# Mr-wang27/llm-inference

Measured on AMD Instinct MI355X. Metric: decode tokens/sec Llama-2-7B fp16 @1 GPU; % HBM roofline; 1->8 TP curve, higher is better.
Workload: dtype fp16; 1 GPU; Llama-2-7B fp16 single-stream greedy decode to 2048 tokens (BASELINE.json configs[1]); TP over n_gpus when > 1; batch=1, prompt=8, ctx=1..2048, kv_cache=f16, weights=fp16, fp32 activations/accumulate, parallelism=single

## Files before the change

### llm-inference_amd/csrc/attn.hip

```cpp
#include <cstdlib>

#include "attn_impl.h"
#include "xchg_impl.h"

namespace llmi {
namespace {

using namespace attn_detail;

template <typename KT, bool HOST_SIZED>
__global__ __launch_bounds__(kThreads) void attn_decode_kernel(AttnArgs a, int ns) {
    extern __shared__ __attribute__((aligned(16))) float smem[];
    WgStamp ts(a.stamps);
    attn_body<KT, PlainIO, HOST_SIZED>(a, blockIdx.x, blockIdx.y, ns, smem, &ts);
}

__global__ __launch_bounds__(kThreads) void attn_merge_kernel(AttnArgs a, int ns) {
    __shared__ float m_s[kMaxSplits];
    __shared__ float l_s[kMaxSplits];
    __shared__ float red_s[16];
    __shared__ float o_red[2][D];
    const int pos = a.pos_dev ? *a.pos_dev : a.pos_host;
    const int h = blockIdx.x, tid = threadIdx.x;
    const int d = tid % D, half = tid / D;
    Ws ws = ws_carve(a.workspace, a.heads, ns);
    const float* mlh = ws.ml + (size_t)h * ns * 2;
    const float* oh = ws.o + (size_t)h * ns * D + d;
    float ov[kMergeChunk];
#pragma unroll
// ... 16 lines not shown
    const float L = block_sum(lw, red_s);
    float O = 0.f;
#pragma unroll
    for (int i = 0; i < kMergeChunk; ++i) {
        const int sp = half + 2 * i;
        const float w = sp < nact ? expf(m_s[sp] - M) : 0.f;
        O = fmaf(sp < nact ? ov[i] : 0.f, w, O);
    }
    for (int sp = half + 2 * kMergeChunk; sp < nact; sp += 2) O = fmaf(oh[(size_t)sp * D], expf(m_s[sp] - M), O);
    o_red[half][d] = O;
    __syncthreads();
    if (tid < D) a.out[(size_t)h * D + tid] = (o_red[0][tid] + o_red[1][tid]) / L;
}

template <typename WT, int NPL>
__global__ __launch_bounds__(kThreads) void attn_oproj_kernel(OprojArgs a, int ns) {
    extern __shared__ __attribute__((aligned(16))) float smem[];
    WgStamp ts(a.stamps);
    oproj_body<WT, NPL, PlainIO>(a, blockIdx.x, blockIdx.y, ns, smem);
    xchg_detail::xchg_tail(a.xt, a.xt_cnt, reinterpret_cast<int*>(smem));
}

template <typename WT, int NPL>
__global__ __launch_bounds__(kThreads) void attn_oproj2_kernel(OprojArgs a, int ns) {
    extern __shared__ __attribute__((aligned(16))) float smem[];
    WgStamp ts(a.stamps);
    oproj_body2<WT, NPL, PlainIO>(a, blockIdx.x, blockIdx.y, ns, smem);
    xchg_detail::xchg_tail(a.xt, a.xt_cnt, reinterpret_cast<int*>(smem));
}

#ifndef LLMI_OPROJ_HG
#define LLMI_OPROJ_HG 2
#endif

int oproj_npl(const OprojArgs& a) {
    const long target = (long)a.heads * a.n_rows / (1024 * 16);
#ifdef LLMI_OPROJ_NPL
    if (target >= 8) return LLMI_OPROJ_NPL;
#endif
    return target >= 8 ? 8 : target >= 4 ? 4 : target >= 2 ? 2 : 1;
}

template <typename WT>
int oproj_launch_w(const OprojArgs& a, hipStream_t s) {
    const int ns = (a.max_seq + CH - 1) / CH;
    const int npl = oproj_npl(a);
    if (LLMI_OPROJ_HG == 2 && sizeof(WT) == 2 && a.heads % 2 == 0 && !a.head_major && npl == 8) {
        const dim3 grid2(a.heads / 2, (a.n_rows + 8 * npl - 1) / (8 * npl));
        hipLaunchKernelGGL((attn_oproj2_kernel<WT, 8>), grid2, dim3(kThreads), oproj2_lds<8>(), s, a, ns);
        LLMI_HIP(hipGetLastError());
        return LLMI_OK;
    }
    const dim3 grid(a.heads, (a.n_rows + 16 * npl - 1) / (16 * npl));
    switch (npl) {
#if LLMI_OPROJ_NPL == 16
        case 16: hipLaunchKernelGGL((attn_oproj_kernel<WT, 16>), grid, dim3(kThreads), oproj_lds<16>(), s, a, ns); break;
#endif
        case 8: hipLaunchKernelGGL((attn_oproj_kernel<WT, 8>), grid, dim3(kThreads), oproj_lds<8>(), s, a, ns); break;
        case 4: hipLaunchKernelGGL((attn_oproj_kernel<WT, 4>), grid, dim3(kThreads), oproj_lds<4>(), s, a, ns); break;
        case 2: hipLaunchKernelGGL((attn_oproj_kernel<WT, 2>), grid, dim3(kThreads), oproj_lds<2>(), s, a, ns); break;
        default: hipLaunchKernelGGL((attn_oproj_kernel<WT, 1>), grid, dim3(kThreads), oproj_lds<1>(), s, a, ns); break;
    }
    LLMI_HIP(hipGetLastError());
    return LLMI_OK;
}

}

size_t attn_workspace_bytes(int heads, int head_dim, int max_seq) {
    (void)head_dim;
    return ws_bytes(heads, max_seq);
}

int attn_decode_launch(const AttnArgs& a, hipStream_t s) {
    LLMI_REQUIRE(a.head_dim == D, "attn: head_dim must be 128");
    LLMI_REQUIRE(a.heads > 0 && a.kv_heads > 0 && a.heads % a.kv_heads == 0, "attn: bad head counts");
    LLMI_REQUIRE(a.max_seq > 0 && (a.max_seq + CH - 1) / CH <= kMaxSplits, "attn: max_seq out of range");
    LLMI_REQUIRE(a.pos_dev || (a.pos_host >= 0 && a.pos_host < a.max_seq), "attn: pos out of range");
    LLMI_REQUIRE(a.qkv && a.k_cache && a.v_cache && a.workspace, "attn: null pointer");
    LLMI_REQUIRE(!a.direct_out || a.out, "attn: null output");
    LLMI_REQUIRE(!a.xacc || a.resid || a.resid_fixed, "attn: xacc seeding needs resid");
    const int ns = (a.max_seq + CH - 1) / CH;
    LLMI_REQUIRE(a.nact >= 0 && a.nact <= ns, "attn: nact out of range");
    LLMI_REQUIRE(a.pos_dev || a.nact == 0 || a.nact == a.pos_host / CH + 1, "attn: nact != ceil((pos + 1) / 64)");
    LLMI_REQUIRE(a.nact == 0 || a.pos_dev, "attn: nact > 0 needs the device position");
    const bool hs = a.nact > 0;
    const dim3 grid(a.heads, hs ? a.nact : ns);
    if (a.cache_dtype == LLMI_F16) {
        if (hs)
            hipLaunchKernelGGL((attn_decode_kernel<__half, true>), grid, dim3(kThreads), kAttnLds, s, a, ns);
        else
            hipLaunchKernelGGL((attn_decode_kernel<__half, false>), grid, dim3(kThreads), kAttnLds, s, a, ns);
    } else if (a.cache_dtype == LLMI_F32) {
        if (hs)
            hipLaunchKernelGGL((attn_decode_kernel<float, true>), grid, dim3(kThreads), kAttnLds, s, a, ns);
        else
            hipLaunchKernelGGL((attn_decode_kernel<float, false>), grid, dim3(kThreads), kAttnLds, s, a, ns);
    } else {
        LLMI_REQUIRE(false, "attn: cache dtype must be f16 or f32");
    }
    LLMI_HIP(hipGetLastError());
    if (a.direct_out) {
        hipLaunchKernelGGL(attn_merge_kernel, dim3(a.heads), dim3(kThreads), 0, s, a, ns);
        LLMI_HIP(hipGetLastError());
    }
    return LLMI_OK;
}

int attn_oproj_launch(const OprojArgs& a, hipStream_t s) {
    LLMI_REQUIRE(a.head_dim == D, "attn_oproj: head_dim must be 128");
    LLMI_REQUIRE(a.w && a.workspace && a.xacc && a.heads > 0 && a.n_rows > 0, "attn_oproj: bad arguments");
    LLMI_REQUIRE(a.ldw >= a.heads * D, "attn_oproj: ldw < heads * head_dim");
// ... 15 lines not shown
```

### llm-inference_amd/csrc/attn_impl.h

```cpp
#pragma once
#include "io.h"
#include "kernels.h"

namespace llmi {
namespace attn_detail {


constexpr int kThreads = 256;
constexpr int D = 128;
#ifndef LLMI_ATTN_CH
#define LLMI_ATTN_CH 64
#endif
constexpr int CH = LLMI_ATTN_CH;
static_assert(CH % 64 == 0 && CH >= kAttnChunk, "chunk must be a multiple of 64");
constexpr int LPR = 16;

constexpr int NPG = CH / (kThreads / LPR);
constexpr int kMaxSplits = 1024;
constexpr int kMergeChunk = 16;
static_assert(kThreads == 2 * D, "merge maps two threads to each head dim");

__device__ __forceinline__ float block_max(float v, float* red) {
    const int lane = threadIdx.x & 63, w = threadIdx.x >> 6, nw = (blockDim.x + 63) >> 6;
    v = wave_max(v);
// ... 100 lines not shown
    } else {
        Raw<float> f;
        f.v[0] = r.v[0];
        f.v[1] = r.v[1];
        unpack8(f, v);
    }
}

constexpr size_t kAttnLds = (3 * D + CH + (kThreads / LPR) * D + 4) * sizeof(float);

__device__ __forceinline__ unsigned long long ld_granule(const unsigned long long* p) {
    return __hip_atomic_load(p, __ATOMIC_RELAXED, __HIP_MEMORY_SCOPE_AGENT);
}

template <typename KT, typename IO, bool HOST_SIZED = false, bool TAGGED = false>
__device__ __forceinline__ void attn_body(const AttnArgs& a, int h, int split, int ns, float* smem,
                                          const WgStamp* ts = nullptr) {
    static_assert(!TAGGED || HOST_SIZED, "the fused launch sizes the attention grid on the host");
    float* q_s = smem;
    float* kcur_s = q_s + D;
    float* vcur_s = kcur_s + D;
    float* p_s = vcur_s + D;
    float (*o_red)[D] = reinterpret_cast<float (*)[D]>(p_s + CH);
    float* ml_s = p_s + CH + (kThreads / LPR) * D;

    const int group = a.heads / a.kv_heads;
    const int kvh = h / group;
    const int tid = threadIdx.x;
    const int grp = tid / LPR, l16 = tid % LPR;
    const int start = split * CH;
    KT* kc = reinterpret_cast<KT*>(a.k_cache) + (size_t)kvh * a.max_seq * D;
// ... 243 lines not shown
        for (int i = h * per + tid; i < min((h + 1) * per, a.hidden); i += kThreads) {
            const bool pre = HOST_SIZED && a.resid_fixed && i == h * per + (int)tid;
            IO::st_ll(a.xacc + i, a.resid_scale == 0.f ? 0ll
                                  : pre            ? psd
                                  : a.resid_fixed  ? a.resid_fixed[i]
                                                   : to_fixed(a.resid[i]));
        }
    }
}


template <int NPL>
constexpr size_t oproj_lds() { return (2 * kMaxSplits + 4 + D + 2 * D + 16 * NPL) * sizeof(float); }

template <typename WT, int NPL>
__device__ __forceinline__ void oproj_load_w(const OprojArgs& a, int h, int chunk, W8<WT> (&wr)[NPL]) {
    const int grp = threadIdx.x / LPR, l16 = threadIdx.x % LPR;
    const int row0 = chunk * 16 * NPL;
    const WT* w = reinterpret_cast<const WT*>(a.w);
#pragma unroll
    for (int t = 0; t < NPL; ++t) {
        int row = row0 + grp + 16 * t;
        row = row < a.n_rows ? row : a.n_rows - 1;
        const size_t off = a.head_major ? ((size_t)h * a.n_rows + row) * D : (size_t)row * a.ldw + (size_t)h * D;
        if constexpr (sizeof(WT) == 1 && NPL >= 2) {
            if (t < NPL / 2) {
                int r2 = row0 + grp + 16 * (2 * t + (l16 >> 3));
                r2 = r2 < a.n_rows ? r2 : a.n_rows - 1;
                const size_t off2 =
                    a.head_major ? ((size_t)h * a.n_rows + r2) * D : (size_t)r2 * a.ldw + (size_t)h * D;
                wr[t].v[0] = ld_nt16(w + off2 + (l16 & 7) * 16);
            }
        } else {
            wr[t] = ld_w8<WT>(w + off + l16 * 8);
        }
    }
}

template <typename WT, int NPL, typename IO>
__device__ __forceinline__ void oproj_body(const OprojArgs& a, int h, int chunk, int ns, float* smem) {
    float* m_s = smem;
    float* l_s = m_s + kMaxSplits;
    float& linv_s = l_s[kMaxSplits];
    float* o_s = l_s + kMaxSplits + 4;
    float (*o_red)[D] = reinterpret_cast<float (*)[D]>(o_s + D);
    float* y_s = o_s + 3 * D;
    const int tid = threadIdx.x;
    const int grp = tid / LPR, l16 = tid % LPR;
    const int row0 = chunk * 16 * NPL;
    const WT* w = reinterpret_cast<const WT*>(a.w);

    Ws ws = ws_carve(const_cast<void*>(a.workspace), a.heads, ns);
    const int d = tid % D, half = tid / D;
    const float* mlh = ws.ml + (size_t)h * ns * 2;
    const float* oh = ws.o + (size_t)h * ns * D + d;
// ... 98 lines not shown
            atomicAdd(reinterpret_cast<unsigned long long*>(a.xacc + row), (unsigned long long)to_fixed(v));
        }
    }
}


template <int NPL>
constexpr size_t oproj2_lds() { return (4 * kMaxSplits + 4 + 2 * D + 2 * 8 * NPL) * sizeof(float); }

__device__ __forceinline__ float ld_wt(const float* p) {
    return __uint_as_float(__hip_atomic_load(reinterpret_cast<const unsigned*>(p), __ATOMIC_RELAXED,
                                             __HIP_MEMORY_SCOPE_AGENT));
}

template <typename WT, int NPL, typename IO, bool FUSED = false>
__device__ __forceinline__ void oproj_body2(const OprojArgs& a, int hp, int chunk, int ns, float* smem) {
    float* m_s = smem;
    float* l_s = m_s + 2 * kMaxSplits;
    float* linv_s = l_s + 2 * kMaxSplits;
    float* o_s = linv_s + 4;
    float* y_s = o_s + 2 * D;
    const int tid = threadIdx.x;
    const int grp = tid / LPR, l16 = tid % LPR;
    const int hs = grp >> 3, g8 = grp & 7;
    const int h = 2 * hp + hs;
    const int row0 = chunk * 8 * NPL;
    const WT* w = reinterpret_cast<const WT*>(a.w);

    Ws ws = ws_carve(const_cast<void*>(a.workspace), a.heads, ns);
    const int mh = tid >> 7, d = tid & (D - 1);
    const float* mlh = ws.ml + (size_t)(2 * hp + mh) * ns * 2;
// ... 162 lines not shown
```

### llm-inference_amd/csrc/common.h

```cpp
#pragma once
#include <hip/hip_runtime.h>
#include <hip/hip_fp16.h>
#include <cstdint>
#include <cstdio>
#include <cstring>
#include <string>
#include <stdexcept>

#include "../../include/llmi.h"

namespace llmi {

constexpr int kWave = 64;

void set_last_error(const std::string& msg);

struct Status {
    int code = LLMI_OK;
};

#define LLMI_HIP(expr)                                                                 \
    do {                                                                               \
        hipError_t _e = (expr);                                                        \
        if (_e != hipSuccess) {                                                        \
// ... 128 lines not shown

constexpr int kLo8Exp = 12;
__device__ __forceinline__ uint32_t lo8_pack4(float l0, float l1, float l2, float l3) {
    auto c = [](float v) { return fminf(fmaxf(v * (float)(1 << kLo8Exp), -448.f), 448.f); };
    int r = __builtin_amdgcn_cvt_pk_fp8_f32(c(l0), c(l1), 0, false);
    r = __builtin_amdgcn_cvt_pk_fp8_f32(c(l2), c(l3), r, true);
    return (uint32_t)r;
}

struct WgStamp {
    unsigned long long* p;
    unsigned long long t0;
    __device__ __forceinline__ explicit WgStamp(unsigned long long* base)
        : p(base ? base + 8 * ((size_t)blockIdx.x + (size_t)gridDim.x * blockIdx.y) : nullptr),
          t0(base ? __builtin_amdgcn_s_memrealtime() : 0ull) {}
    __device__ __forceinline__ void mark(int i) const {
        if (p && threadIdx.x == 0) p[i] = __builtin_amdgcn_s_memrealtime();
    }
    __device__ __forceinline__ ~WgStamp() {
        if (p && threadIdx.x == 0) {
            p[0] = t0;
            p[3] = __builtin_amdgcn_s_memrealtime();
            p[4] = __smid();
        }
    }
};

}
```

### llm-inference_amd/csrc/gemv_impl.h

```cpp
#pragma once
#include "io.h"
#include "kernels.h"

namespace llmi {
namespace gemv_detail {

constexpr int kThreads = 256;
constexpr int kWavesPerBlock = kThreads / kWave;
#ifndef LLMI_GEMV_UNROLL
#define LLMI_GEMV_UNROLL 8
#endif
#ifndef LLMI_GEMV_ROWS
#define LLMI_GEMV_ROWS 2
#endif
#ifndef LLMI_I8_PIPE
#define LLMI_I8_PIPE 0
#endif
#ifndef LLMI_GEMV_PIPE16
#define LLMI_GEMV_PIPE16 0
#endif
constexpr int kUnrollMax = LLMI_GEMV_UNROLL;
constexpr int kRows = LLMI_GEMV_ROWS;

template <typename WT> struct WT_ { };
// ... 70 lines not shown
}

inline int gemv_pick_unroll(int epl, int epi, const GemvArgs& a, int groups) {
    const int kl = (epi == EPI_ATOMIC) ? a.k / a.ksplit : a.k;
    const int nc = kl / epl / (a.kpar > 1 ? a.kpar : 1);
    auto slots = [&](int u) { const int b = kWave * u; return (nc + b - 1) / b * b; };
    if (a.kpar > 1) return 4;
    int best = (epi != EPI_ARGMAX && groups >= 4096 && groups <= 12288 && kUnrollMax >= 4) ? 4 : kUnrollMax;
    for (int u : {4, 5, 8})
        if (u <= kUnrollMax && slots(u) < slots(best)) best = u;
    return best;
}

template <typename WT, int ROWS, int EPI, bool NORM, typename GT, int XPT, int kUnroll, bool XFIX, typename IO,
          int KPT = 1, bool TAG = false>
__device__ __forceinline__ void gemv_body(const GemvArgs& a, int bid, int nblk, float4* xs) {
    static_assert(!TAG || EPI == EPI_STORE, "granule rows: store epilogue only");
    const unsigned long long tag_hi = TAG ? (unsigned long long)(*a.tag_epoch * 128u + a.tag_layer) << 32 : 0ull;
    auto seed = [&, bid0 = bid, nblk0 = nblk]() {
        if (a.seed_dst == nullptr) return;
        const int per = (a.seed_n + nblk0 - 1) / nblk0;
        const int i0 = bid0 * per, i1 = min(i0 + per, a.seed_n);
        for (int i = i0 + (int)threadIdx.x; i < i1; i += kThreads)
            IO::st_ll(a.seed_dst + i, a.seed_keep ? IO::ld_ll(a.seed_src + i) : 0ll);
    };
    constexpr int EPL = WT_<WT>::EPL;
    constexpr int PK = EPL / 4;
    static_assert(!(XFIX && EPI == EPI_ATOMIC), "split-K reads an fp32 x");
    const int S = (EPI == EPI_ATOMIC) ? a.ksplit : 1;
    const int ks = bid % S;
    bid /= S;
// ... 2 lines not shown
    const int k4 = k / 4;
    const int nc = k / EPL;
    float* red = reinterpret_cast<float*>(xs + k4);
    unsigned long long* best_s = reinterpret_cast<unsigned long long*>(red + 16);
    float* kpart = reinterpret_cast<float*>(best_s + kWavesPerBlock);
    const int tid = threadIdx.x, lane = tid & 63;
    const int n_groups = (EPI == EPI_SILU_MUL) ? a.pair_off : (a.n_rows + ROWS - 1) / ROWS;
    constexpr bool PIPE = (sizeof(WT) == 1 && kUnroll <= 5 && ((LLMI_I8_PIPE >> EPI) & 1))
                          || (sizeof(WT) == 2 && ((LLMI_GEMV_PIPE16 >> EPI) & 1));
    constexpr bool KPOK = (EPI == EPI_STORE || EPI == EPI_SILU_MUL) && ROWS <= 2 && !PIPE;
    constexpr int KP = KPOK ? KPT : 1;
    const int wave = (tid >> 6) / KP, kq = (tid >> 6) % KP;
    constexpr int gpw = kWavesPerBlock / KP;
    const int c_lo = KP > 1 ? kq * (nc / KP) : 0;
    const int c_hi = KP > 1 ? c_lo + nc / KP : nc;
    const size_t row_bytes = (size_t)(a.ldw ? a.ldw : a.k) * sizeof(WT);
    const char* wbase = reinterpret_cast<const char*>(a.w) + (size_t)ks * k * sizeof(WT);
    const float4* x4 = reinterpret_cast<const float4*>(a.x + (size_t)ks * k);

    auto rows_of = [&](int g, int* rows) {
        if constexpr (TAG) {
            if (a.tag_heads > 0) {
                const int h = g / 192, rem = g - 192 * h, t = rem >> 6;
                g = t * a.tag_heads * 64 + h * 64 + (rem & 63);
            }
        }
#pragma unroll
        for (int r = 0; r < ROWS; ++r) rows[r] = (EPI == EPI_SILU_MUL) ? g + r * a.pair_off : g * ROWS + r;
    };
    auto load_batch = [&](uint4 (&wv)[ROWS][kUnroll], const int* rows, int base) {
#pragma unroll
// ... 252 lines not shown
```

### llm-inference_amd/csrc/gemv_launch.h

```cpp
#pragma once
#include "gemv_impl.h"
#include "xchg_impl.h"

namespace llmi {
namespace gemv_detail {


#ifndef LLMI_GEMV_MAX_GRID
#define LLMI_GEMV_MAX_GRID 1024
#endif
#ifndef LLMI_GEMV_MIN_WAVES
#define LLMI_GEMV_MIN_WAVES 1
#endif

#ifndef LLMI_GEMV_MIN_WAVES_I8
#define LLMI_GEMV_MIN_WAVES_I8 4
#endif
template <typename WT, int U> constexpr int min_waves() {
    return sizeof(WT) == 1 && U <= 5 ? LLMI_GEMV_MIN_WAVES_I8 : LLMI_GEMV_MIN_WAVES;
}

template <typename WT, int ROWS, int EPI, bool NORM, typename GT, int XPT, int kUnroll, bool XFIX, int KPT = 1>
__global__ __launch_bounds__(kThreads, (min_waves<WT, kUnroll>())) void gemv_kernel(GemvArgs a) {
    extern __shared__ __attribute__((aligned(16))) float4 xs[];
    WgStamp ts(a.stamps);
    gemv_body<WT, ROWS, EPI, NORM, GT, XPT, kUnroll, XFIX, PlainIO, KPT>(a, blockIdx.x, gridDim.x, xs);
    if constexpr (EPI == EPI_ATOMIC || EPI == EPI_ARGMAX) {
        const int k4 = (EPI == EPI_ATOMIC ? a.k / a.ksplit : a.k) / 4;
        xchg_detail::xchg_tail(a.xt, a.xt_cnt, reinterpret_cast<int*>(xs + k4) + 15);
    }
}

inline int device_cus() {
    static int cus = 0;
    if (cus == 0) {
        int dev = 0;
        if (hipGetDevice(&dev) != hipSuccess ||
            hipDeviceGetAttribute(&cus, hipDeviceAttributeMultiprocessorCount, dev) != hipSuccess)
            cus = 0;
    }
    return cus;
// ... 3 lines not shown
    auto kern = gemv_kernel<WT, ROWS, EPI, NORM, GT, XPT, U, XF, KPT>;
    if (EPI != EPI_ARGMAX && a.grid == 0 && a.kpar <= 1) {
        static size_t occ_lds = ~(size_t)0;
        static int occ_blocks = 0;
        if (lds != occ_lds) {
            int n = 0;
            if (hipOccupancyMaxActiveBlocksPerMultiprocessor(&n, reinterpret_cast<const void*>(kern), kThreads, lds) !=
                hipSuccess)
                n = 0;
            occ_blocks = n * device_cus();
            occ_lds = lds;
        }
        const int S = (EPI == EPI_ATOMIC) ? a.ksplit : 1;
        if (occ_blocks >= S && grid > occ_blocks) grid = occ_blocks / S * S;
    }
    hipLaunchKernelGGL(kern, dim3(grid), dim3(kThreads), lds, s, a);
    LLMI_HIP(hipGetLastError());
    return LLMI_OK;
}

template <typename WT, int ROWS, int EPI, bool NORM, typename GT, int U, bool XF>
int launch_u(const GemvArgs& a, int grid, hipStream_t s) {
    const int kl = (EPI == EPI_ATOMIC) ? a.k / a.ksplit : a.k;
    const size_t lds = gemv_lds_bytes(kl);
    const int k4 = kl / 4;
    const int xpt = gemv_xpt(k4);
    if constexpr ((EPI == EPI_STORE || EPI == EPI_SILU_MUL) && NORM && XF && U == 4) {
        if (a.kpar > 1) {
            LLMI_REQUIRE(k4 <= 5 * kThreads, "gemv: kpar needs k <= 5120");
            if (a.kpar == 2)
                return xpt == 4 ? launch_k<WT, ROWS, EPI, NORM, GT, 4, U, XF, 2>(a, grid, lds, s)
// ... 66 lines not shown
```

### llm-inference_amd/csrc/ops.hip

```cpp
#include <cmath>
#include <cstring>

#include <algorithm>

#include "kernels.h"
#include "prng.h"

namespace llmi {
namespace {

constexpr int kT = 256;

template <typename T>
__device__ __forceinline__ float ld(const void* p, size_t i) {
    return to_f32(reinterpret_cast<const T*>(p)[i]);
}
__device__ __forceinline__ float ldg(const void* p, int dt, size_t i) {
    return dt == LLMI_F16 ? ld<__half>(p, i) : ld<float>(p, i);
}

template <typename TT>
__global__ void embedding_kernel(const int32_t* ids, const TT* table, int vocab, int hidden, float* out,
                                 int* err) {
    const int t = blockIdx.y;
// ... 112 lines not shown
        unsigned long long k = argmax_key(logits[i], (uint32_t)i);
        best = k > best ? k : best;
    }
    best = block_max_key(best, sh);
    if (threadIdx.x == 0) partials[blockIdx.x] = best;
}

__global__ void argmax_final_kernel(const unsigned long long* partials, int np, int32_t* out) {
    __shared__ unsigned long long sh[16];
    unsigned long long best = 0;
    for (int i = threadIdx.x; i < np; i += blockDim.x) best = partials[i] > best ? partials[i] : best;
    best = block_max_key(best, sh);
    if (threadIdx.x == 0) *out = (int32_t)argmax_key_index(best);
}

template <typename TT>
__global__ void step_start_kernel(DecodeState* st, const int32_t* prompt, const unsigned long long* partials,
                                  int np, int32_t* tokens, const TT* table, int hidden, float* x,
                                  long long* xres, int max_seq, unsigned* cnt, int cnt_words, long long* xres2) {
    __shared__ unsigned long long sh[16];
    for (int i = threadIdx.x; i < cnt_words; i += blockDim.x) cnt[i] = 0u;
    __shared__ int tok_s;
    const int p = st->next_pos;
    if (p >= max_seq) {
        if (threadIdx.x == 0) {
            atomicOr(&st->error, 2);
            st->epoch = st->epoch + 1u;
        }
        return;
    }
    int tok;
    if (p < st->prompt_len) {
        tok = prompt[p];
    } else {
        unsigned long long best = 0;
        for (int i = threadIdx.x; i < np; i += blockDim.x) best = partials[i] > best ? partials[i] : best;
        best = block_max_key(best, sh);
        tok = (int)argmax_key_index(best);
    }
    if (threadIdx.x == 0) {
        if (tok < 0 || tok >= st->vocab) {
            atomicOr(&st->error, 1);
            tok = 0;
        }
        tok_s = tok;
    }
    __syncthreads();
    tok = tok_s;
    if (threadIdx.x == 0) {
        tokens[p] = tok;
        st->cur_pos = p;
        st->next_pos = p + 1;
        st->epoch = st->epoch + 1u;
    }
    const TT* row = table + (size_t)tok * hidden;
    for (int i = threadIdx.x; i < hidden; i += blockDim.x) {
        const float v = to_f32(row[i]);
        x[i] = v;
        if (xres) xres[i] = to_fixed(v);
        if (xres2) xres2[i] = to_fixed(v);
    }
}

__global__ void finalize_kernel(DecodeState* st, const unsigned long long* partials, int np, int32_t* tokens,
                                int max_seq) {
    __shared__ unsigned long long sh[16];
    const int p = st->next_pos;
    unsigned long long best = 0;
    for (int i = threadIdx.x; i < np; i += blockDim.x) best = partials[i] > best ? partials[i] : best;
    best = block_max_key(best, sh);
    if (threadIdx.x == 0 && p <= max_seq && p >= st->prompt_len) tokens[p] = (int)argmax_key_index(best);
// ... 237 lines not shown
    return LLMI_OK;
}

int argmax_launch(const float* logits, int n, int32_t* out_id, unsigned long long* scratch, hipStream_t s) {
    LLMI_REQUIRE(logits && out_id && scratch && n > 0, "argmax: bad arguments");
    const int grid = std::min((n + kT - 1) / kT, 256);
    hipLaunchKernelGGL(argmax_partial_kernel, dim3(grid), dim3(kT), 0, s, logits, n, scratch);
    hipLaunchKernelGGL(argmax_final_kernel, dim3(1), dim3(kT), 0, s, scratch, grid, out_id);
    LLMI_HIP(hipGetLastError());
    return LLMI_OK;
}

int step_start_launch(DecodeState* st, const int32_t* prompt, const unsigned long long* partials, int np,
                      int32_t* tokens, const void* table, int t_dtype, int hidden, float* x, long long* xres,
                      int max_seq, unsigned* cnt, int cnt_words, hipStream_t s, long long* xres2) {
    if (t_dtype == LLMI_F16)
        hipLaunchKernelGGL(step_start_kernel<__half>, dim3(1), dim3(1024), 0, s, st, prompt, partials, np, tokens,
                           (const __half*)table, hidden, x, xres, max_seq, cnt, cnt ? cnt_words : 0, xres2);
    else
        hipLaunchKernelGGL(step_start_kernel<float>, dim3(1), dim3(1024), 0, s, st, prompt, partials, np, tokens,
                           (const float*)table, hidden, x, xres, max_seq, cnt, cnt ? cnt_words : 0, xres2);
    LLMI_HIP(hipGetLastError());
    return LLMI_OK;
}

int finalize_launch(DecodeState* st, const unsigned long long* partials, int np, int32_t* tokens, int max_seq,
                    hipStream_t s) {
    hipLaunchKernelGGL(finalize_kernel, dim3(1), dim3(1024), 0, s, st, partials, np, tokens, max_seq);
    LLMI_HIP(hipGetLastError());
    return LLMI_OK;
}

__global__ void group_reduce_kernel(void* const* bufs, int W, int n, int op) {
    const int i = blockIdx.x * blockDim.x + threadIdx.x;
    if (i >= n) return;
    if (op == 0) {
// ... 47 lines not shown
```

### llm-inference_amd/csrc/qkv_attn.hip

```cpp
#include "attn_impl.h"
#include "gemv_launch.h"

#ifndef LLMI_QA_MINW_SPILL
#define LLMI_QA_MINW_SPILL 3
#endif
template <typename WT, int U> constexpr int qa_minw() {
    return (sizeof(WT) >= 2 && U == 4) || sizeof(WT) == 4 ? 4 : LLMI_QA_MINW_SPILL;
}

namespace llmi {
namespace {

int qa_grid_cap = 0;
int qa_order = 1;
int qa_poll_all = 0;

template <typename WT, typename GT, int XPT, int U, typename KT, bool WITH_O>
__global__ __launch_bounds__(256, (qa_minw<WT, U>())) void qkv_attn_kernel(GemvArgs g, AttnArgs at, OprojArgs o,
                                                                            int g_grid, int ns) {
    extern __shared__ __attribute__((aligned(16))) float4 xs[];
    WgStamp ts(g.stamps);
    if constexpr (WITH_O) {
        const int ob = (int)blockIdx.x - g_grid - at.heads * at.nact;
        if (ob >= 0) {
            const int n_chunks = (o.n_rows + 63) / 64;
            attn_detail::oproj_body2<WT, 8, PlainIO, true>(o, ob / n_chunks, ob % n_chunks, ns,
                                                           reinterpret_cast<float*>(xs));
            return;
        }
    }
    if ((int)blockIdx.x < g_grid) {
        gemv_detail::gemv_body<WT, gemv_detail::kRows, EPI_STORE, true, GT, XPT, U, true, PlainIO, 1, true>(
            g, blockIdx.x, g_grid, xs);
    } else {
        const int b = (int)blockIdx.x - g_grid;
        const int h = g.tag_heads > 0 ? b / at.nact : b % at.heads;
        const int sp = g.tag_heads > 0 ? b - h * at.nact : b / at.heads;
        attn_detail::attn_body<KT, PlainIO, true, true>(at, h, sp, ns, reinterpret_cast<float*>(xs), &ts);
    }
}

template <typename WT, typename GT, int XPT, int U, typename KT, bool WITH_O>
int launch_k(const GemvArgs& g, const AttnArgs& at, const OprojArgs* o, hipStream_t s) {
    auto kern = qkv_attn_kernel<WT, GT, XPT, U, KT, WITH_O>;
    size_t lds = std::max(gemv_detail::gemv_lds_bytes(g.k), attn_detail::kAttnLds);
    if (WITH_O) lds = std::max(lds, attn_detail::oproj2_lds<8>());
    int G = gemv_grid(g);
    static size_t occ_lds = ~(size_t)0;
    static int occ_blocks = 0;
    if (lds != occ_lds) {
        int n = 0;
        if (hipOccupancyMaxActiveBlocksPerMultiprocessor(&n, reinterpret_cast<const void*>(kern), 256, lds) != hipSuccess)
// ... 3 lines not shown
    }
    if (occ_blocks > 0 && G > occ_blocks) G = occ_blocks;
    if (qa_grid_cap > 0 && qa_grid_cap < G) G = qa_grid_cap;
    const int ns = (at.max_seq + attn_detail::CH - 1) / attn_detail::CH;
    int grid = G + at.heads * at.nact;
    GemvArgs gg = g;
    AttnArgs aa = at;
    OprojArgs oo;
    gg.tag_heads = (qa_order && at.heads == at.kv_heads && g.n_rows == 3 * at.heads * attn_detail::D) ? at.heads : 0;
    aa.tag_poll_all = qa_poll_all;
    if (WITH_O) {
        oo = *o;
        aa.publish = 1;
        grid += (at.heads / 2) * ((o->n_rows + 63) / 64);
    }
    hipLaunchKernelGGL(kern, dim3(grid), dim3(256), lds, s, gg, aa, oo, G, ns);
    LLMI_HIP(hipGetLastError());
    return LLMI_OK;
}

template <typename WT, typename GT, int XPT, int U>
int launch_kt(const GemvArgs& g, const AttnArgs& at, const OprojArgs* o, hipStream_t s) {
    if constexpr (sizeof(WT) == 2 && XPT == 4 && U == 4) {
        if (o)
            return at.cache_dtype == LLMI_F16 ? launch_k<WT, GT, XPT, U, __half, true>(g, at, o, s)
                                              : launch_k<WT, GT, XPT, U, float, true>(g, at, o, s);
    }
    return at.cache_dtype == LLMI_F16 ? launch_k<WT, GT, XPT, U, __half, false>(g, at, nullptr, s)
                                      : launch_k<WT, GT, XPT, U, float, false>(g, at, nullptr, s);
}

// ... 85 lines not shown
```

Baseline: 380.2 tokens/s.

## Pack kernel arguments into cache-line hot/cold structs and pin hot fields in SGPRs

Replaces the large GemvArgs/AttnArgs/OprojArgs kernel parameters with packed structs whose first 64-byte line holds the fields every workgroup reads, with rarely used fields in a cold tail. Empty inline asm with "s" constraints forces the hot fields to be loaded into scalar registers at kernel entry, and derived values (ns, nblk, ldw default) are precomputed on the host. The intent is to shrink kernarg fetch latency at workgroup start for these short decode kernels. The cost is extra host-side packing and possible SGPR pressure from the pinned values.

```diff
diff --git a/llm-inference_amd/csrc/attn.hip b/llm-inference_amd/csrc/attn.hip
--- a/llm-inference_amd/csrc/attn.hip
+++ b/llm-inference_amd/csrc/attn.hip
@@ -9,10 +9,11 @@
 using namespace attn_detail;
 
 template <typename KT, bool HOST_SIZED>
-__global__ __launch_bounds__(kThreads) void attn_decode_kernel(AttnArgs a, int ns) {
+__global__ __launch_bounds__(kThreads) void attn_decode_kernel(AttnK a) {
     extern __shared__ __attribute__((aligned(16))) float smem[];
-    WgStamp ts(a.stamps);
-    attn_body<KT, PlainIO, HOST_SIZED>(a, blockIdx.x, blockIdx.y, ns, smem, &ts);
+    pin_hot(a);
+    WgStamp ts(a.stamps, (size_t)blockIdx.x + (size_t)a.heads * blockIdx.y);
+    attn_body<KT, PlainIO, HOST_SIZED>(a, blockIdx.x, blockIdx.y, a.ns, smem, &ts);
 }
 
 __global__ __launch_bounds__(kThreads) void attn_merge_kernel(AttnArgs a, int ns) {
@@ -59,18 +60,20 @@
 }
 
 template <typename WT, int NPL>
-__global__ __launch_bounds__(kThreads) void attn_oproj_kernel(OprojArgs a, int ns) {
+__global__ __launch_bounds__(kThreads) void attn_oproj_kernel(OprojK a) {
     extern __shared__ __attribute__((aligned(16))) float smem[];
-    WgStamp ts(a.stamps);
-    oproj_body<WT, NPL, PlainIO>(a, blockIdx.x, blockIdx.y, ns, smem);
+    pin_hot(a);
+    WgStamp ts(a.stamps, (size_t)blockIdx.x + (size_t)a.nblk_x * blockIdx.y);
+    oproj_body<WT, NPL, PlainIO>(a, blockIdx.x, blockIdx.y, a.ns, smem);
     xchg_detail::xchg_tail(a.xt, a.xt_cnt, reinterpret_cast<int*>(smem));
 }
 
 template <typename WT, int NPL>
-__global__ __launch_bounds__(kThreads) void attn_oproj2_kernel(OprojArgs a, int ns) {
+__global__ __launch_bounds__(kThreads) void attn_oproj2_kernel(OprojK a) {
     extern __shared__ __attribute__((aligned(16))) float smem[];
-    WgStamp ts(a.stamps);
-    oproj_body2<WT, NPL, PlainIO>(a, blockIdx.x, blockIdx.y, ns, smem);
+    pin_hot(a);
+    WgStamp ts(a.stamps, (size_t)blockIdx.x + (size_t)a.nblk_x * blockIdx.y);
+    oproj_body2<WT, NPL, PlainIO>(a, blockIdx.x, blockIdx.y, a.ns, smem);
     xchg_detail::xchg_tail(a.xt, a.xt_cnt, reinterpret_cast<int*>(smem));
 }
 
@@ -92,19 +95,21 @@
     const int npl = oproj_npl(a);
     if (LLMI_OPROJ_HG == 2 && sizeof(WT) == 2 && a.heads % 2 == 0 && !a.head_major && npl == 8) {
         const dim3 grid2(a.heads / 2, (a.n_rows + 8 * npl - 1) / (8 * npl));
-        hipLaunchKernelGGL((attn_oproj2_kernel<WT, 8>), grid2, dim3(kThreads), oproj2_lds<8>(), s, a, ns);
+        hipLaunchKernelGGL((attn_oproj2_kernel<WT, 8>), grid2, dim3(kThreads), oproj2_lds<8>(), s,
+                           oproj_pack(a, ns, (int)grid2.x));
         LLMI_HIP(hipGetLastError());
         return LLMI_OK;
     }
     const dim3 grid(a.heads, (a.n_rows + 16 * npl - 1) / (16 * npl));
+    const OprojK k = oproj_pack(a, ns, (int)grid.x);
     switch (npl) {
 #if LLMI_OPROJ_NPL == 16
-        case 16: hipLaunchKernelGGL((attn_oproj_kernel<WT, 16>), grid, dim3(kThreads), oproj_lds<16>(), s, a, ns); break;
+        case 16: hipLaunchKernelGGL((attn_oproj_kernel<WT, 16>), grid, dim3(kThreads), oproj_lds<16>(), s, k); break;
 #endif
-        case 8: hipLaunchKernelGGL((attn_oproj_kernel<WT, 8>), grid, dim3(kThreads), oproj_lds<8>(), s, a, ns); break;
-        case 4: hipLaunchKernelGGL((attn_oproj_kernel<WT, 4>), grid, dim3(kThreads), oproj_lds<4>(), s, a, ns); break;
-        case 2: hipLaunchKernelGGL((attn_oproj_kernel<WT, 2>), grid, dim3(kThreads), oproj_lds<2>(), s, a, ns); break;
-        default: hipLaunchKernelGGL((attn_oproj_kernel<WT, 1>), grid, dim3(kThreads), oproj_lds<1>(), s, a, ns); break;
+        case 8: hipLaunchKernelGGL((attn_oproj_kernel<WT, 8>), grid, dim3(kThreads), oproj_lds<8>(), s, k); break;
+        case 4: hipLaunchKernelGGL((attn_oproj_kernel<WT, 4>), grid, dim3(kThreads), oproj_lds<4>(), s, k); break;
+        case 2: hipLaunchKernelGGL((attn_oproj_kernel<WT, 2>), grid, dim3(kThreads), oproj_lds<2>(), s, k); break;
+        default: hipLaunchKernelGGL((attn_oproj_kernel<WT, 1>), grid, dim3(kThreads), oproj_lds<1>(), s, k); break;
     }
     LLMI_HIP(hipGetLastError());
     return LLMI_OK;
@@ -131,16 +136,17 @@
     LLMI_REQUIRE(a.nact == 0 || a.pos_dev, "attn: nact > 0 needs the device position");
     const bool hs = a.nact > 0;
     const dim3 grid(a.heads, hs ? a.nact : ns);
+    const AttnK k = attn_pack(a, ns, false);
     if (a.cache_dtype == LLMI_F16) {
         if (hs)
-            hipLaunchKernelGGL((attn_decode_kernel<__half, true>), grid, dim3(kThreads), kAttnLds, s, a, ns);
+            hipLaunchKernelGGL((attn_decode_kernel<__half, true>), grid, dim3(kThreads), kAttnLds, s, k);
         else
-            hipLaunchKernelGGL((attn_decode_kernel<__half, false>), grid, dim3(kThreads), kAttnLds, s, a, ns);
+            hipLaunchKernelGGL((attn_decode_kernel<__half, false>), grid, dim3(kThreads), kAttnLds, s, k);
     } else if (a.cache_dtype == LLMI_F32) {
         if (hs)
-            hipLaunchKernelGGL((attn_decode_kernel<float, true>), grid, dim3(kThreads), kAttnLds, s, a, ns);
+            hipLaunchKernelGGL((attn_decode_kernel<float, true>), grid, dim3(kThreads), kAttnLds, s, k);
         else
-            hipLaunchKernelGGL((attn_decode_kernel<float, false>), grid, dim3(kThreads), kAttnLds, s, a, ns);
+            hipLaunchKernelGGL((attn_decode_kernel<float, false>), grid, dim3(kThreads), kAttnLds, s, k);
     } else {
         LLMI_REQUIRE(false, "attn: cache dtype must be f16 or f32");
     }
diff --git a/llm-inference_amd/csrc/attn_impl.h b/llm-inference_amd/csrc/attn_impl.h
--- a/llm-inference_amd/csrc/attn_impl.h
+++ b/llm-inference_amd/csrc/attn_impl.h
@@ -1,5 +1,6 @@
 #pragma once
 #include "io.h"
+#include "kargs.h"
 #include "kernels.h"
 
 namespace llmi {
@@ -138,7 +139,7 @@
 }
 
 template <typename KT, typename IO, bool HOST_SIZED = false, bool TAGGED = false>
-__device__ __forceinline__ void attn_body(const AttnArgs& a, int h, int split, int ns, float* smem,
+__device__ __forceinline__ void attn_body(const AttnK& a, int h, int split, int ns, float* smem,
                                           const WgStamp* ts = nullptr) {
     static_assert(!TAGGED || HOST_SIZED, "the fused launch sizes the attention grid on the host");
     float* q_s = smem;
@@ -412,7 +413,7 @@
 constexpr size_t oproj_lds() { return (2 * kMaxSplits + 4 + D + 2 * D + 16 * NPL) * sizeof(float); }
 
 template <typename WT, int NPL>
-__device__ __forceinline__ void oproj_load_w(const OprojArgs& a, int h, int chunk, W8<WT> (&wr)[NPL]) {
+__device__ __forceinline__ void oproj_load_w(const OprojK& a, int h, int chunk, W8<WT> (&wr)[NPL]) {
     const int grp = threadIdx.x / LPR, l16 = threadIdx.x % LPR;
     const int row0 = chunk * 16 * NPL;
     const WT* w = reinterpret_cast<const WT*>(a.w);
@@ -436,7 +437,7 @@
 }
 
 template <typename WT, int NPL, typename IO>
-__device__ __forceinline__ void oproj_body(const OprojArgs& a, int h, int chunk, int ns, float* smem) {
+__device__ __forceinline__ void oproj_body(const OprojK& a, int h, int chunk, int ns, float* smem) {
     float* m_s = smem;
     float* l_s = m_s + kMaxSplits;
     float& linv_s = l_s[kMaxSplits];
@@ -565,7 +566,7 @@
 }
 
 template <typename WT, int NPL, typename IO, bool FUSED = false>
-__device__ __forceinline__ void oproj_body2(const OprojArgs& a, int hp, int chunk, int ns, float* smem) {
+__device__ __forceinline__ void oproj_body2(const OprojK& a, int hp, int chunk, int ns, float* smem) {
     float* m_s = smem;
     float* l_s = m_s + 2 * kMaxSplits;
     float* linv_s = l_s + 2 * kMaxSplits;
diff --git a/llm-inference_amd/csrc/common.h b/llm-inference_amd/csrc/common.h
--- a/llm-inference_amd/csrc/common.h
+++ b/llm-inference_amd/csrc/common.h
@@ -166,6 +166,8 @@
     __device__ __forceinline__ explicit WgStamp(unsigned long long* base)
         : p(base ? base + 8 * ((size_t)blockIdx.x + (size_t)gridDim.x * blockIdx.y) : nullptr),
           t0(base ? __builtin_amdgcn_s_memrealtime() : 0ull) {}
+    __device__ __forceinline__ WgStamp(unsigned long long* base, size_t block)
+        : p(base ? base + 8 * block : nullptr), t0(base ? __builtin_amdgcn_s_memrealtime() : 0ull) {}
     __device__ __forceinline__ void mark(int i) const {
         if (p && threadIdx.x == 0) p[i] = __builtin_amdgcn_s_memrealtime();
     }
diff --git a/llm-inference_amd/csrc/gemv_impl.h b/llm-inference_amd/csrc/gemv_impl.h
--- a/llm-inference_amd/csrc/gemv_impl.h
+++ b/llm-inference_amd/csrc/gemv_impl.h
@@ -1,5 +1,6 @@
 #pragma once
 #include "io.h"
+#include "kargs.h"
 #include "kernels.h"
 
 namespace llmi {
@@ -108,7 +109,7 @@
 
 template <typename WT, int ROWS, int EPI, bool NORM, typename GT, int XPT, int kUnroll, bool XFIX, typename IO,
           int KPT = 1, bool TAG = false>
-__device__ __forceinline__ void gemv_body(const GemvArgs& a, int bid, int nblk, float4* xs) {
+__device__ __forceinline__ void gemv_body(const GemvK& a, int bid, int nblk, float4* xs) {
     static_assert(!TAG || EPI == EPI_STORE, "granule rows: store epilogue only");
     const unsigned long long tag_hi = TAG ? (unsigned long long)(*a.tag_epoch * 128u + a.tag_layer) << 32 : 0ull;
     auto seed = [&, bid0 = bid, nblk0 = nblk]() {
@@ -141,7 +142,7 @@
     constexpr int gpw = kWavesPerBlock / KP;
     const int c_lo = KP > 1 ? kq * (nc / KP) : 0;
     const int c_hi = KP > 1 ? c_lo + nc / KP : nc;
-    const size_t row_bytes = (size_t)(a.ldw ? a.ldw : a.k) * sizeof(WT);
+    const size_t row_bytes = (size_t)a.ldw * sizeof(WT);
     const char* wbase = reinterpret_cast<const char*>(a.w) + (size_t)ks * k * sizeof(WT);
     const float4* x4 = reinterpret_cast<const float4*>(a.x + (size_t)ks * k);
 
diff --git a/llm-inference_amd/csrc/gemv_launch.h b/llm-inference_amd/csrc/gemv_launch.h
--- a/llm-inference_amd/csrc/gemv_launch.h
+++ b/llm-inference_amd/csrc/gemv_launch.h
@@ -21,10 +21,11 @@
 }
 
 template <typename WT, int ROWS, int EPI, bool NORM, typename GT, int XPT, int kUnroll, bool XFIX, int KPT = 1>
-__global__ __launch_bounds__(kThreads, (min_waves<WT, kUnroll>())) void gemv_kernel(GemvArgs a) {
+__global__ __launch_bounds__(kThreads, (min_waves<WT, kUnroll>())) void gemv_kernel(GemvK a) {
     extern __shared__ __attribute__((aligned(16))) float4 xs[];
-    WgStamp ts(a.stamps);
-    gemv_body<WT, ROWS, EPI, NORM, GT, XPT, kUnroll, XFIX, PlainIO, KPT>(a, blockIdx.x, gridDim.x, xs);
+    pin_hot(a);
+    WgStamp ts(a.stamps, blockIdx.x);
+    gemv_body<WT, ROWS, EPI, NORM, GT, XPT, kUnroll, XFIX, PlainIO, KPT>(a, blockIdx.x, a.nblk, xs);
     if constexpr (EPI == EPI_ATOMIC || EPI == EPI_ARGMAX) {
         const int k4 = (EPI == EPI_ATOMIC ? a.k / a.ksplit : a.k) / 4;
         xchg_detail::xchg_tail(a.xt, a.xt_cnt, reinterpret_cast<int*>(xs + k4) + 15);
@@ -58,7 +59,7 @@
         const int S = (EPI == EPI_ATOMIC) ? a.ksplit : 1;
         if (occ_blocks >= S && grid > occ_blocks) grid = occ_blocks / S * S;
     }
-    hipLaunchKernelGGL(kern, dim3(grid), dim3(kThreads), lds, s, a);
+    hipLaunchKernelGGL(kern, dim3(grid), dim3(kThreads), lds, s, gemv_pack(a, grid));
     LLMI_HIP(hipGetLastError());
     return LLMI_OK;
 }
diff --git a/llm-inference_amd/csrc/kargs.h b/llm-inference_amd/csrc/kargs.h
--- /dev/null
+++ b/llm-inference_amd/csrc/kargs.h
@@ -0,0 +1,287 @@
+#pragma once
+#include "kernels.h"
+
+namespace llmi {
+
+constexpr int kHotLine = 64;
+
+struct alignas(64) GemvHot {
+    union {
+        const float* x;
+        const long long* x_fixed;
+    };
+    const void* gamma;
+    const void* w;
+    float* x_out;
+    unsigned long long* stamps;
+    int k;
+    int n_rows;
+    int ldw;
+    int nblk;
+    union {
+        int pair_off;
+        int ksplit;
+        int tag_heads;
+    };
+    unsigned tag_layer;
+};
+static_assert(sizeof(GemvHot) == kHotLine, "the GEMV's hot block is one line");
+
+struct GemvCold {
+    const unsigned* tag_epoch;
+    float eps;
+    float resid_scale;
+    const __half* scales;
+    float* y;
+    const float* resid;
+    unsigned long long* partials;
+    uint32_t idx_base;
+    int yacc_single;
+    long long* yacc;
+    const long long* yacc_base;
+    long long* yacc_copy;
+    const long long* seed_src;
+    long long* seed_dst;
+    int seed_n;
+    int seed_keep;
+    unsigned long long* y_tag;
+    unsigned* xt_cnt;
+    XchgArgs xt;
+};
+
+struct GemvK : GemvHot, GemvCold {};
+
+inline GemvK gemv_pack(const GemvArgs& a, int nblk) {
+    GemvK k{};
+    if (a.x_fixed) k.x_fixed = a.x_fixed; else k.x = a.x;
+    k.gamma = a.gamma;
+    k.w = a.w;
+    k.x_out = a.x_out;
+    k.stamps = a.stamps;
+    k.k = a.k;
+    k.n_rows = a.n_rows;
+    k.ldw = a.ldw ? a.ldw : a.k;
+    k.nblk = nblk;
+    k.pair_off = a.epi == EPI_SILU_MUL ? a.pair_off : a.epi == EPI_ATOMIC ? a.ksplit : a.tag_heads;
+    k.tag_layer = a.tag_layer;
+    k.tag_epoch = a.tag_epoch;
+    k.eps = a.eps;
+    k.resid_scale = a.resid_scale;
+    k.scales = a.scales;
+    k.y = a.y;
+    k.resid = a.resid;
+    k.partials = a.partials;
+    k.idx_base = a.idx_base;
+    k.yacc_single = a.yacc_single;
+    k.yacc = a.yacc;
+    k.yacc_base = a.yacc_base;
+    k.yacc_copy = a.yacc_copy;
+    k.seed_src = a.seed_src;
+    k.seed_dst = a.seed_dst;
+    k.seed_n = a.seed_n;
+    k.seed_keep = a.seed_keep;
+    k.y_tag = a.y_tag;
+    k.xt_cnt = a.xt_cnt;
+    k.xt = a.xt;
+    return k;
+}
+
+struct alignas(64) AttnHot {
+    const int* pos_dev;
+    void* k_cache;
+    void* v_cache;
+    union {
+        const float* qkv;
+        const unsigned long long* qkv_tag;
+    };
+    unsigned long long* stamps;
+    int heads, kv_heads;
+    int max_seq;
+    int nact;
+    int pos_host;
+    int ns;
+};
+static_assert(sizeof(AttnHot) == kHotLine, "the attention's hot block is one line");
+
+struct AttnCold {
+    const unsigned* tag_epoch;
+    unsigned tag_layer;
+    int tag_poll_all;
+    long long* xacc;
+    const long long* resid_fixed;
+    const float* resid;
+    float resid_scale;
+    int hidden;
+    const float* rope_tab;
+    float rope_base;
+    int rope;
+    float* out;
+    void* workspace;
+    int* err;
+    int direct_out;
+    int publish;
+};
+
+struct AttnK : AttnHot, AttnCold {};
+
+inline AttnK attn_pack(const AttnArgs& a, int ns, bool tagged) {
+    AttnK k{};
+    k.pos_dev = a.pos_dev;
+    k.k_cache = a.k_cache;
+    k.v_cache = a.v_cache;
+    if (tagged) k.qkv_tag = a.qkv_tag; else k.qkv = a.qkv;
+    k.stamps = a.stamps;
+    k.heads = a.heads;
+    k.kv_heads = a.kv_heads;
+    k.max_seq = a.max_seq;
+    k.nact = a.nact;
+    k.pos_host = a.pos_host;
+    k.ns = ns;
+    k.tag_epoch = a.tag_epoch;
+    k.tag_layer = a.tag_layer;
+    k.tag_poll_all = a.tag_poll_all;
+    k.xacc = a.xacc;
+    k.resid_fixed = a.resid_fixed;
+    k.resid = a.resid;
+    k.resid_scale = a.resid_scale;
+    k.hidden = a.hidden;
+    k.rope_tab = a.rope_tab;
+    k.rope_base = a.rope_base;
+    k.rope = a.rope;
+    k.out = a.out;
+    k.workspace = a.workspace;
+    k.err = a.err;
+    k.direct_out = a.direct_out;
+    k.publish = a.publish;
+    return k;
+}
+
+struct alignas(64) OprojHot {
+    const void* workspace;
+    const void* w;
+    unsigned long long* stamps;
+    int heads;
+    int ns;
+    int nact;
+    int n_rows, ldw;
+    int head_major;
+    int nblk_x;
+};
+static_assert(sizeof(OprojHot) == kHotLine, "the o_proj's hot block is one line");
+
+struct OprojCold {
+    const __half* scales;
+    long long* xacc;
+    const int* pos_dev;
+    int pos_host;
+    int max_seq;
+    int* err;
+    unsigned* xt_cnt;
+    XchgArgs xt;
+};
+
+struct OprojK : OprojHot, OprojCold {};
+
+inline OprojK oproj_pack(const OprojArgs& a, int ns, int nblk_x) {
+    OprojK k{};
+    k.workspace = a.workspace;
+    k.w = a.w;
+    k.stamps = a.stamps;
+    k.heads = a.heads;
+    k.ns = ns;
+    k.nact = a.nact;
+    k.n_rows = a.n_rows;
+    k.ldw = a.ldw;
+    k.head_major = a.head_major;
+    k.nblk_x = nblk_x;
+    k.scales = a.scales;
+    k.xacc = a.xacc;
+    k.pos_dev = a.pos_dev;
+    k.pos_host = a.pos_host;
+    k.max_seq = a.max_seq;
+    k.err = a.err;
+    k.xt_cnt = a.xt_cnt;
+    k.xt = a.xt;
+    return k;
+}
+
+struct alignas(64) QkvAttnHot1 {
+    const int* pos_dev;
+    void* k_cache;
+    void* v_cache;
+    const unsigned long long* qkv_tag;
+    const unsigned* tag_epoch;
+    int heads, kv_heads;
+    int max_seq;
+    int nact;
+    int ns;
+};
+static_assert(sizeof(QkvAttnHot1) == kHotLine, "the fused launch's second hot line");
+
+struct QkvAttnK {
+    GemvHot gh;
+    QkvAttnHot1 h1;
+    GemvCold gc;
+    AttnCold ac;
+    OprojK o;
+};
+
+inline QkvAttnK qkv_attn_pack(const GemvArgs& g, int g_grid, const AttnArgs& at, int ns, const OprojArgs& o,
+                              int grid) {
+    QkvAttnK q{};
+    const GemvK gk = gemv_pack(g, g_grid);
+    const AttnK ak = attn_pack(at, ns, true);
+    q.gh = gk;
+    q.gc = gk;
+    q.ac = ak;
+    q.h1.pos_dev = at.pos_dev;
+    q.h1.k_cache = at.k_cache;
+    q.h1.v_cache = at.v_cache;
+    q.h1.qkv_tag = at.qkv_tag;
+    q.h1.tag_epoch = g.tag_epoch;
+    q.h1.heads = at.heads;
+    q.h1.kv_heads = at.kv_heads;
+    q.h1.max_seq = at.max_seq;
+    q.h1.nact = at.nact;
+    q.h1.ns = ns;
+    q.o = oproj_pack(o, ns, grid);
+    return q;
+}
+
+struct alignas(64) StepStartK {
+    DecodeState* st;
+    unsigned* cnt;
+    const int32_t* prompt;
+    const unsigned long long* partials;
+    int32_t* tokens;
+    const void* table;
+    int cnt_words;
+    int max_seq;
+    int np;
+    int hidden;
+    float* x;
+    long long* xres;
+    long long* xres2;
+};
+static_assert(sizeof(StepStartK) == 2 * kHotLine, "step_start: one hot line, one cold");
+
+#ifdef __HIPCC__
+__device__ __forceinline__ void pin_hot(const GemvHot& h) {
+    asm volatile("" ::"s"(h.x), "s"(h.gamma), "s"(h.w), "s"(h.x_out), "s"(h.stamps), "s"(h.k), "s"(h.n_rows),
+                 "s"(h.ldw), "s"(h.nblk), "s"(h.pair_off), "s"(h.tag_layer));
+}
+__device__ __forceinline__ void pin_hot(const AttnHot& h) {
+    asm volatile("" ::"s"(h.pos_dev), "s"(h.k_cache), "s"(h.v_cache), "s"(h.qkv), "s"(h.stamps), "s"(h.heads),
+                 "s"(h.kv_heads), "s"(h.max_seq), "s"(h.nact), "s"(h.pos_host), "s"(h.ns));
+}
+__device__ __forceinline__ void pin_hot(const QkvAttnHot1& h) {
+    asm volatile("" ::"s"(h.pos_dev), "s"(h.k_cache), "s"(h.v_cache), "s"(h.qkv_tag), "s"(h.tag_epoch), "s"(h.heads),
+                 "s"(h.kv_heads), "s"(h.max_seq), "s"(h.nact), "s"(h.ns));
+}
+__device__ __forceinline__ void pin_hot(const OprojHot& h) {
+    asm volatile("" ::"s"(h.workspace), "s"(h.w), "s"(h.stamps), "s"(h.heads), "s"(h.ns), "s"(h.nact), "s"(h.n_rows),
+                 "s"(h.ldw), "s"(h.head_major), "s"(h.nblk_x));
+}
+#endif
+
+}
diff --git a/llm-inference_amd/csrc/ops.hip b/llm-inference_amd/csrc/ops.hip
--- a/llm-inference_amd/csrc/ops.hip
+++ b/llm-inference_amd/csrc/ops.hip
@@ -3,6 +3,7 @@
 
 #include <algorithm>
 
+#include "kargs.h"
 #include "kernels.h"
 #include "prng.h"
 
@@ -150,12 +151,24 @@
     if (threadIdx.x == 0) *out = (int32_t)argmax_key_index(best);
 }
 
+constexpr int kStepThreads = 1024;
+
 template <typename TT>
-__global__ void step_start_kernel(DecodeState* st, const int32_t* prompt, const unsigned long long* partials,
-                                  int np, int32_t* tokens, const TT* table, int hidden, float* x,
-                                  long long* xres, int max_seq, unsigned* cnt, int cnt_words, long long* xres2) {
+__global__ __launch_bounds__(kStepThreads) void step_start_kernel(StepStartK a) {
+    asm volatile("" ::"s"(a.st), "s"(a.cnt), "s"(a.prompt), "s"(a.partials), "s"(a.tokens), "s"(a.table),
+                 "s"(a.cnt_words), "s"(a.max_seq), "s"(a.np), "s"(a.hidden));
+    DecodeState* st = a.st;
+    const int32_t* prompt = a.prompt;
+    const unsigned long long* partials = a.partials;
+    int32_t* tokens = a.tokens;
+    const TT* table = static_cast<const TT*>(a.table);
+    unsigned* cnt = a.cnt;
+    const int cnt_words = a.cnt_words, max_seq = a.max_seq, np = a.np, hidden = a.hidden;
+    float* x = a.x;
+    long long* xres = a.xres;
+    long long* xres2 = a.xres2;
     __shared__ unsigned long long sh[16];
-    for (int i = threadIdx.x; i < cnt_words; i += blockDim.x) cnt[i] = 0u;
+    for (int i = threadIdx.x; i < cnt_words; i += kStepThreads) cnt[i] = 0u;
     __shared__ int tok_s;
     const int p = st->next_pos;
     if (p >= max_seq) {
@@ -170,7 +183,7 @@
         tok = prompt[p];
     } else {
         unsigned long long best = 0;
-        for (int i = threadIdx.x; i < np; i += blockDim.x) best = partials[i] > best ? partials[i] : best;
+        for (int i = threadIdx.x; i < np; i += kStepThreads) best = partials[i] > best ? partials[i] : best;
         best = block_max_key(best, sh);
         tok = (int)argmax_key_index(best);
     }
@@ -190,7 +203,7 @@
         st->epoch = st->epoch + 1u;
     }
     const TT* row = table + (size_t)tok * hidden;
-    for (int i = threadIdx.x; i < hidden; i += blockDim.x) {
+    for (int i = threadIdx.x; i < hidden; i += kStepThreads) {
         const float v = to_f32(row[i]);
         x[i] = v;
         if (xres) xres[i] = to_fixed(v);
@@ -458,12 +471,24 @@
 int step_start_launch(DecodeState* st, const int32_t* prompt, const unsigned long long* partials, int np,
                       int32_t* tokens, const void* table, int t_dtype, int hidden, float* x, long long* xres,
                       int max_seq, unsigned* cnt, int cnt_words, hipStream_t s, long long* xres2) {
+    StepStartK a{};
+    a.st = st;
+    a.cnt = cnt;
+    a.prompt = prompt;
+    a.partials = partials;
+    a.tokens = tokens;
+    a.table = table;
+    a.cnt_words = cnt ? cnt_words : 0;
+    a.max_seq = max_seq;
+    a.np = np;
+    a.hidden = hidden;
+    a.x = x;
+    a.xres = xres;
+    a.xres2 = xres2;
     if (t_dtype == LLMI_F16)
-        hipLaunchKernelGGL(step_start_kernel<__half>, dim3(1), dim3(1024), 0, s, st, prompt, partials, np, tokens,
-                           (const __half*)table, hidden, x, xres, max_seq, cnt, cnt ? cnt_words : 0, xres2);
+        hipLaunchKernelGGL(step_start_kernel<__half>, dim3(1), dim3(kStepThreads), 0, s, a);
     else
-        hipLaunchKernelGGL(step_start_kernel<float>, dim3(1), dim3(1024), 0, s, st, prompt, partials, np, tokens,
-                           (const float*)table, hidden, x, xres, max_seq, cnt, cnt ? cnt_words : 0, xres2);
+        hipLaunchKernelGGL(step_start_kernel<float>, dim3(1), dim3(kStepThreads), 0, s, a);
     LLMI_HIP(hipGetLastError());
     return LLMI_OK;
 }
diff --git a/llm-inference_amd/csrc/qkv_attn.hip b/llm-inference_amd/csrc/qkv_attn.hip
--- a/llm-inference_amd/csrc/qkv_attn.hip
+++ b/llm-inference_amd/csrc/qkv_attn.hip
@@ -16,26 +16,47 @@
 int qa_poll_all = 0;
 
 template <typename WT, typename GT, int XPT, int U, typename KT, bool WITH_O>
-__global__ __launch_bounds__(256, (qa_minw<WT, U>())) void qkv_attn_kernel(GemvArgs g, AttnArgs at, OprojArgs o,
-                                                                            int g_grid, int ns) {
+__global__ __launch_bounds__(256, (qa_minw<WT, U>())) void qkv_attn_kernel(QkvAttnK q) {
     extern __shared__ __attribute__((aligned(16))) float4 xs[];
-    WgStamp ts(g.stamps);
+    pin_hot(q.gh);
+    pin_hot(q.h1);
+    const int g_grid = q.gh.nblk, ns = q.h1.ns;
+    WgStamp ts(q.gh.stamps, blockIdx.x);
     if constexpr (WITH_O) {
-        const int ob = (int)blockIdx.x - g_grid - at.heads * at.nact;
+        const int ob = (int)blockIdx.x - g_grid - q.h1.heads * q.h1.nact;
         if (ob >= 0) {
-            const int n_chunks = (o.n_rows + 63) / 64;
-            attn_detail::oproj_body2<WT, 8, PlainIO, true>(o, ob / n_chunks, ob % n_chunks, ns,
+            const int n_chunks = (q.o.n_rows + 63) / 64;
+            attn_detail::oproj_body2<WT, 8, PlainIO, true>(q.o, ob / n_chunks, ob % n_chunks, ns,
                                                            reinterpret_cast<float*>(xs));
             return;
         }
     }
     if ((int)blockIdx.x < g_grid) {
+        GemvK g;
+        static_cast<GemvHot&>(g) = q.gh;
+        static_cast<GemvCold&>(g) = q.gc;
+        g.tag_epoch = q.h1.tag_epoch;
         gemv_detail::gemv_body<WT, gemv_detail::kRows, EPI_STORE, true, GT, XPT, U, true, PlainIO, 1, true>(
             g, blockIdx.x, g_grid, xs);
     } else {
+        AttnK at;
+        static_cast<AttnCold&>(at) = q.ac;
+        at.pos_dev = q.h1.pos_dev;
+        at.k_cache = q.h1.k_cache;
+        at.v_cache = q.h1.v_cache;
+        at.qkv_tag = q.h1.qkv_tag;
+        at.stamps = q.gh.stamps;
+        at.heads = q.h1.heads;
+        at.kv_heads = q.h1.kv_heads;
+        at.max_seq = q.h1.max_seq;
+        at.nact = q.h1.nact;
+        at.pos_host = 0;
+        at.ns = ns;
+        at.tag_epoch = q.h1.tag_epoch;
+        at.tag_layer = q.gh.tag_layer;
         const int b = (int)blockIdx.x - g_grid;
-        const int h = g.tag_heads > 0 ? b / at.nact : b % at.heads;
-        const int sp = g.tag_heads > 0 ? b - h * at.nact : b / at.heads;
+        const int h = q.gh.tag_heads > 0 ? b / at.nact : b % at.heads;
+        const int sp = q.gh.tag_heads > 0 ? b - h * at.nact : b / at.heads;
         attn_detail::attn_body<KT, PlainIO, true, true>(at, h, sp, ns, reinterpret_cast<float*>(xs), &ts);
     }
 }
@@ -69,7 +90,7 @@
         aa.publish = 1;
         grid += (at.heads / 2) * ((o->n_rows + 63) / 64);
     }
-    hipLaunchKernelGGL(kern, dim3(grid), dim3(256), lds, s, gg, aa, oo, G, ns);
+    hipLaunchKernelGGL(kern, dim3(grid), dim3(256), lds, s, qkv_attn_pack(gg, G, aa, ns, oo, grid));
     LLMI_HIP(hipGetLastError());
     return LLMI_OK;
 }
```

Measured after the change: 381.5 tokens/s (median of 6 runs). Within noise of the previous version (+0.4%).
